# nghorbani/moshpp

Measured on NVIDIA H100. Metric: mocap frames solved/sec (Stage-II), higher is better.
Workload: dtype f32

## Files before the change

### moshpp_b200/csrc/mosh2_device.cuh

```cuda
#pragma once
#include <math.h>
#include <stdint.h>

#if defined(__CUDACC__) && !defined(MOSH2_EMU)
#define M2_HD __host__ __device__ __forceinline__
#define M2_D __device__ __forceinline__
#define M2_NOINLINE __device__ __noinline__
#define M2_SYNC() __syncthreads()
#define M2_WSYNC() __syncwarp()
#define M2_GPU 1
#else
#define M2_HD inline
#define M2_D inline
#define M2_NOINLINE static inline
#define M2_SYNC() ((void)0)
#define M2_WSYNC() ((void)0)
#define M2_GPU 0
#endif

#if defined(MOSH2_PROFILE) && M2_GPU
#define M2_T0() long long t_prev_ = clock64()
#define M2_TACC(slot) do { if (cta.tid == 0) { const long long t_now_ = clock64(); w.prof[(slot) + prof_base] += t_now_ - t_prev_; t_prev_ = t_now_; } } while (0)
#define M2_TRESET() do { t_prev_ = clock64(); } while (0)
#else
// ... 297 lines not shown
    SPtr<real> red, sc, hct;
    SPtr<int> colmap, colsrc, jlist, isc;
    SPtr<int> st_colmap, st_colsrc, st_jlist, st_meta;
    SPtr<int> c_parents, c_fk_order, c_wj, c_free1, c_free2, c_pids;
    SPtr<int> c_tin, c_tsz;
    SPtr<real> c_wv, c_v0, c_coefs, c_j0, c_hmean, c_pmeans, c_pnlw;
    SPtr<real> c_jd;
    SPtr<long long> prof;
    SPtr<uint8_t> vis;
    SPtr<uint32_t> c_chain;
    SPtr<uint8_t> c_amask;
    SPtr<unsigned long long> mbar;
    uint32_t stage_ofs, stage_bytes;
    int tc_ok;
    int tc;
};

constexpr int kMaxDepth = 16;
constexpr int kDR = 28;
constexpr int kM3 = 12;
#if M2_GPU
namespace tc {
__device__ __forceinline__ uint32_t smem_u32(const void *p) { return static_cast<uint32_t>(__cvta_generic_to_shared(p)); }
__device__ __forceinline__ uint32_t to_tf32(float v) { uint32_t r; asm("cvt.rna.tf32.f32 %0, %1;" : "=r"(r) : "f"(v)); return r; }
__device__ __forceinline__ void mma_tf32_m16n8k8(float (&d)[4], const uint32_t (&a)[4], uint32_t b0, uint32_t b1) {
    asm volatile("mma.sync.aligned.m16n8k8.row.col.f32.tf32.tf32.f32 {%0, %1, %2, %3}, {%4, %5, %6, %7}, {%8, %9}, {%0, %1, %2, %3};"
                 : "+f"(d[0]), "+f"(d[1]), "+f"(d[2]), "+f"(d[3]) : "r"(a[0]), "r"(a[1]), "r"(a[2]), "r"(a[3]), "r"(b0), "r"(b1));
}
__device__ __forceinline__ void jtj_block_tf32(const float *J, int ld, int rows, int cols, int i0, int j0,
                                               float (&hh)[2][4], float (&cr)[2][4]) {
    const int lane = threadIdx.x & 31, g = lane >> 2, t = lane & 3;
    const int ca0 = i0 + g, ca1 = i0 + 8 + g, cb0 = j0 + g, cb1 = j0 + 8 + g;
    for (int k0 = 0; k0 < rows; k0 += 8) {
        const int k1 = k0 + t, k2 = k0 + t + 4;
        const float *r1 = J + (k1 < rows ? k1 : 0) * ld, *r2 = J + (k2 < rows ? k2 : 0) * ld;
        const bool in1 = k1 < rows, in2 = k2 < rows;
        const float av[4] = {(in1 && ca0 < cols) ? r1[ca0] : 0.f, (in1 && ca1 < cols) ? r1[ca1] : 0.f,
                             (in2 && ca0 < cols) ? r2[ca0] : 0.f, (in2 && ca1 < cols) ? r2[ca1] : 0.f};
        const float bv[2][2] = {{(in1 && cb0 < cols) ? r1[cb0] : 0.f, (in2 && cb0 < cols) ? r2[cb0] : 0.f},
                                {(in1 && cb1 < cols) ? r1[cb1] : 0.f, (in2 && cb1 < cols) ? r2[cb1] : 0.f}};
        uint32_t ahi[4], alo[4], bhi[2][2], blo[2][2];
#pragma unroll
        for (int q = 0; q < 4; ++q) { ahi[q] = to_tf32(av[q]); alo[q] = to_tf32(av[q] - __uint_as_float(ahi[q])); }
#pragma unroll
        for (int nj = 0; nj < 2; ++nj)
#pragma unroll
            for (int q = 0; q < 2; ++q) { bhi[nj][q] = to_tf32(bv[nj][q]); blo[nj][q] = to_tf32(bv[nj][q] - __uint_as_float(bhi[nj][q])); }
#pragma unroll
        for (int nj = 0; nj < 2; ++nj) {
            mma_tf32_m16n8k8(hh[nj], ahi, bhi[nj][0], bhi[nj][1]);
            mma_tf32_m16n8k8(cr[nj], alo, bhi[nj][0], bhi[nj][1]);
            mma_tf32_m16n8k8(cr[nj], ahi, blo[nj][0], blo[nj][1]);
            mma_tf32_m16n8k8(cr[nj], alo, blo[nj][0], blo[nj][1]);
        }
    }
}
__device__ __forceinline__ void mbar_init(uint32_t mbar, uint32_t count) {
    asm volatile("mbarrier.init.shared::cta.b64 [%0], %1;" :: "r"(mbar), "r"(count) : "memory");
    asm volatile("fence.mbarrier_init.release.cluster;" ::: "memory");
}
__device__ __forceinline__ void mbar_wait(uint32_t mbar, uint32_t parity) {
    asm volatile("{\n\t.reg .pred p;\n\tWAIT_%=:\n\t"
                 "mbarrier.try_wait.parity.shared::cta.b64 p, [%0], %1;\n\t"
                 "@p bra DONE_%=;\n\tbra WAIT_%=;\n\tDONE_%=:\n\t}\n" :: "r"(mbar), "r"(parity) : "memory");
}
__device__ __forceinline__ void mbar_expect_tx(uint32_t mbar, uint32_t bytes) {
    asm volatile("mbarrier.arrive.expect_tx.shared::cta.b64 _, [%0], %1;" :: "r"(mbar), "r"(bytes) : "memory");
}
__device__ __forceinline__ void bulk_g2s(uint32_t dst_smem, const void *src, uint32_t bytes, uint32_t mbar) {
    asm volatile("cp.async.bulk.shared::cluster.global.mbarrier::complete_tx::bytes [%0], [%1], %2, [%3];"
                 :: "r"(dst_smem), "l"(src), "r"(bytes), "r"(mbar) : "memory");
}
__device__ __forceinline__ void fence_async_smem() { asm volatile("fence.proxy.async.shared::cta;" ::: "memory"); }
}
#endif

struct Dims {
    int nJ, M, S, PF, PR, nd, NX, NCt, n1, n2, ld, lda, ldp, npad, K, D, D4, kw, jt_size, tmk;
};

template <class real>
M2_HD Dims make_dims(const Model<real> &m) {
    Dims d;
    d.nJ = m.nJ; d.M = m.M; d.S = 3 * m.M; d.PF = 3 * m.nJ; d.PR = m.p_red; d.nd = m.nd;
    d.NX = 3 + m.p_red + m.nd; d.NCt = (m.n_hand_full + 3) & ~3;    d.n1 = m.n1; d.n2 = m.n2;
    d.npad = (m.n2 + 3) & ~3;
    d.ld = ((m.n2 + 7) & ~7) + 4;
    d.ldp = d.npad + 4;
    d.lda = d.npad | 1;
    d.K = m.prior_k; d.D = m.prior_d; d.D4 = m.prior_d4; d.kw = m.kw;
    d.tmk = m.tile_markers > 0 ? m.tile_markers : 10;
    const int a = 3 * d.tmk * d.NCt, b = kBlendGroups * 9 * m.M + 16;
    d.jt_size = a > b ? a : b;
    return d;
}

struct Arena {
    size_t off;
    template <class T> M2_HD uint32_t take(size_t n) {
        off = (off + 15) & ~size_t(15);
        const size_t o = off;
        off += n * sizeof(T);
        return uint32_t(o);
    }
};

template <class real, bool BIG>
M2_HD void carve(Work<real, BIG> &w, const Dims &d, const Model<real> &m, Arena &S, Arena &G) {
    const int hct_size = m.hct_size;
    Arena &B = BIG ? G : S;
    w.x.ofs = S.take<real>(d.NX); w.xt.ofs = S.take<real>(d.NX);
    w.pose_prev.ofs = S.take<real>(d.PR); w.velo_tgt.ofs = S.take<real>(d.PR); w.dm_tgt.ofs = S.take<real>(d.nd + 1);
    w.fullpose.ofs = S.take<real>(d.PF); w.Rl.ofs = S.take<real>(9 * d.nJ); w.dRl.ofs = S.take<real>(kDR * d.nJ);
    w.Jp.ofs = S.take<real>(3 * d.nJ); w.Rg.ofs = S.take<real>(9 * d.nJ); w.tg.ofs = S.take<real>(3 * d.nJ);
    w.vp.ofs = S.take<real>(3 * d.S); w.pj.ofs = S.take<real>(3 * d.S * d.kw); w.Rsk.ofs = S.take<real>(9 * d.S);
    w.mk.ofs = S.take<real>(3 * d.M); w.rm.ofs = S.take<real>(3 * d.M); w.obs.ofs = S.take<real>(3 * d.M);
    w.py.ofs = S.take<real>(d.K * d.D + 1); w.pq.ofs = S.take<real>(d.K + 1); w.pxg.ofs = S.take<real>(d.D + 1);
    {
        w.A.ofs = B.take<real>(size_t(d.n2) * d.lda);
        w.tc_ok = (sizeof(real) == 4 && !BIG && !m.dev_no_tc) ? 1 : 0;
        w.tc = 0;
        const size_t mark_b = B.off;
        w.Lm.ofs = B.take<real>(size_t(d.n2 + 1) * d.ld);
        const size_t end_b = B.off;
        B.off = mark_b;
        w.Jt.ofs = B.take<real>(d.jt_size);
        w.Jf.ofs = B.take<real>(3 * d.tmk * d.npad);
        if (!BIG) {
            w.Loc.ofs = S.take<real>(3 * kM3 * d.M); w.MtR.ofs = S.take<real>(kM3 * d.S);
            w.u.ofs = S.take<real>(kM3 * d.nJ); w.dtg.ofs = S.take<real>(3 * d.nJ * d.nd + 1);
        }
        if (B.off < end_b) B.off = end_b;
    }
    if (BIG) {
        w.Loc.ofs = S.take<real>(3 * kM3 * d.M); w.MtR.ofs = S.take<real>(kM3 * d.S);
        w.u.ofs = S.take<real>(kM3 * d.nJ); w.dtg.ofs = S.take<real>(3 * d.nJ * d.nd + 1);
    }
    w.Linv.ofs = S.take<real>(size_t((d.n2 + kCholNB - 1) / kCholNB) * kCholNB * kCholNB);
    w.Pn.ofs = S.take<real>(size_t(kCholNB) * d.ldp);
    w.g.ofs = S.take<real>(d.npad); w.Ag.ofs = S.take<real>(d.npad); w.dgn.ofs = S.take<real>(d.npad);
    w.d.ofs = S.take<real>(d.npad); w.tmp.ofs = S.take<real>(d.npad); w.ds.ofs = S.take<real>(d.npad);
    w.red.ofs = S.take<real>(8 * 33); w.sc.ofs = S.take<real>(16);
    w.colmap.ofs = S.take<int>(d.NX); w.colsrc.ofs = S.take<int>(d.n2); w.jlist.ofs = S.take<int>(d.nJ); w.isc.ofs = S.take<int>(8);
    w.st_colmap.ofs = S.take<int>(2 * d.NX); w.st_colsrc.ofs = S.take<int>(2 * d.n2); w.st_jlist.ofs = S.take<int>(2 * d.nJ); w.st_meta.ofs = S.take<int>(4);
    w.prof.ofs = S.take<long long>(32);
    w.mbar.ofs = S.take<unsigned long long>(1);
    w.vis.ofs = S.take<uint8_t>(d.M);
    S.off = (S.off + 15) & ~size_t(15);
    w.stage_ofs = uint32_t(S.off);
    w.c_parents.ofs = S.take<int>(d.nJ); w.c_fk_order.ofs = S.take<int>(d.nJ);
    w.c_wj.ofs = S.take<int>(d.S * d.kw); w.c_free1.ofs = S.take<int>(d.n1); w.c_free2.ofs = S.take<int>(d.n2);
    w.c_pids.ofs = S.take<int>(d.D + 1);
    w.c_wv.ofs = S.take<real>(d.S * d.kw); w.c_v0.ofs = S.take<real>(3 * d.S); w.c_coefs.ofs = S.take<real>(3 * d.M);
    w.c_j0.ofs = S.take<real>(3 * d.nJ); w.c_hmean.ofs = S.take<real>(m.n_hand_full + 1);
    w.c_pmeans.ofs = S.take<real>(d.K * d.D + 1); w.c_pnlw.ofs = S.take<real>(d.K + 1);
    w.c_jd.ofs = S.take<real>(size_t(3) * d.nJ * d.nd + 1);
    w.hct.ofs = S.take<real>(hct_size + 4);
    S.off = (S.off + 15) & ~size_t(15);
    w.stage_bytes = uint32_t(S.off) - w.stage_ofs;
    w.c_tin.ofs = S.take<int>(d.nJ); w.c_tsz.ofs = S.take<int>(d.nJ); w.c_amask.ofs = S.take<uint8_t>(size_t(d.S) * d.nJ);
    w.c_chain.ofs = S.take<uint32_t>(size_t(d.nJ) * (kMaxDepth / 4));
}

template <class real, bool BIG, class Put>
inline void stage_image(const Work<real, BIG> &w, const Dims &d, int hct_size, int n_hand_full, Put put) {
    const uint32_t b = w.stage_ofs;
    put(w.c_parents.ofs - b, 0, size_t(d.nJ)); put(w.c_fk_order.ofs - b, 1, size_t(d.nJ));
    put(w.c_wj.ofs - b, 2, size_t(d.S) * d.kw); put(w.c_free1.ofs - b, 3, size_t(d.n1)); put(w.c_free2.ofs - b, 4, size_t(d.n2));
    put(w.c_pids.ofs - b, 5, size_t(d.D));
    put(w.c_wv.ofs - b, 6, size_t(d.S) * d.kw); put(w.c_v0.ofs - b, 7, size_t(3) * d.S); put(w.c_coefs.ofs - b, 8, size_t(3) * d.M);
    put(w.c_j0.ofs - b, 9, size_t(3) * d.nJ); put(w.c_hmean.ofs - b, 10, size_t(n_hand_full));
    put(w.c_pmeans.ofs - b, 11, size_t(d.K) * d.D); put(w.c_pnlw.ofs - b, 12, size_t(d.K));
    put(w.c_jd.ofs - b, 13, size_t(3) * d.nJ * d.nd); put(w.hct.ofs - b, 14, size_t(hct_size));
}

template <class real>
struct StepCfg {
    const int *free;
    int n;
    real wp;
    real e3;
    bool velo, poseH, dm_terms, extrap;
    bool face;
};

template <class real, bool BIG = false>
struct Solver {
    const Model<real> &m;
    const Job<real> &job;
    const Work<real, BIG> &w;
    const Cta cta;
    const Dims &d;
    real wd, wp_frame, wH, wv, wdm, wex, wF, wxp;
    int nvis, njl;
    bool has_velo, has_extrap, hand_free;
    int n_iter, n_eval, n_build, n_min, frame_flags;
    int prof_base = 0;
    bool fwd_at_x = false;
    bool fwd_has_prior = false;
    bool resuming = false;
    real resume_diff = 0;
    int lin_f = -1;

    M2_D Solver(const Model<real> &m_, const Job<real> &j_, const Work<real, BIG> &w_, const Dims &d_, Cta c_)
        : m(m_), job(j_), w(w_), cta(c_), d(d_) {}

#define CTA_FOR(i, n) _Pragma("unroll 1") for (int i = cta.tid; i < (n); i += cta.nthr)

    M2_D void cta_max(real *v) {
#if M2_GPU
        real x = v[0];
#pragma unroll
        for (int o = 16; o > 0; o >>= 1) { const real y = __shfl_xor_sync(0xffffffffu, x, o); x = y > x ? y : x; }
        const int lane = cta.tid & 31, warp = cta.tid >> 5, nwarp = (cta.nthr + 31) >> 5;
        if (lane == 0) w.red[warp] = x;
        __syncthreads();
        if (cta.tid == 0) { real mx = w.red[0]; for (int q = 1; q < nwarp; ++q) mx = w.red[q] > mx ? w.red[q] : mx; w.red[32] = mx; }
        __syncthreads();
        v[0] = w.red[32];
        __syncthreads();
#else
        (void)v;
#endif
    }

    M2_D void fk(int l, int nl) {
        for (int j = l; j < d.nJ; j += nl) {
            uint32_t cw[kMaxDepth / 4];
#pragma unroll
            for (int q = 0; q < kMaxDepth / 4; ++q) cw[q] = w.c_chain[j * (kMaxDepth / 4) + q];
            int prev = int(cw[0] & 255u);
            real R[9], t[3];
#pragma unroll
            for (int i = 0; i < 9; ++i) R[i] = w.Rl[9 * prev + i];
#pragma unroll
            for (int i = 0; i < 3; ++i) t[i] = w.Jp[3 * prev + i];
#pragma unroll
            for (int k = 1; k < kMaxDepth; ++k) {
                const int c = int((cw[k >> 2] >> (8 * (k & 3))) & 255u);
                if (c != 255) {
                    const real *Rc = w.Rl + 9 * c;
                    const real dj[3] = {w.Jp[3 * c] - w.Jp[3 * prev], w.Jp[3 * c + 1] - w.Jp[3 * prev + 1], w.Jp[3 * c + 2] - w.Jp[3 * prev + 2]};
                    real rc[9], o[9];
#pragma unroll
                    for (int i = 0; i < 9; ++i) rc[i] = Rc[i];
#pragma unroll
                    for (int i = 0; i < 3; ++i) t[i] += R[3 * i] * dj[0] + R[3 * i + 1] * dj[1] + R[3 * i + 2] * dj[2];
                    mat3_mul_reg(R, rc, o);
#pragma unroll
                    for (int i = 0; i < 9; ++i) R[i] = o[i];
                    prev = c;
                }
            }
#pragma unroll
            for (int i = 0; i < 9; ++i) w.Rg[9 * j + i] = R[i];
#pragma unroll
            for (int i = 0; i < 3; ++i) w.tg[3 * j + i] = t[i];
        }
    }

    M2_D int blend_groups(int nl) const {
        const int per_group = 3 * ((d.S + 3) >> 2);
        int g = nl / per_group;
        return g < 1 ? 1 : (g > kBlendGroups ? kBlendGroups : g);
    }
    M2_D void blend_partials(int l, int nl) {
        const int G = blend_groups(nl);
        const int per = (d.nJ - 1 + G - 1) / G;
        const int Sq = (d.S + 3) >> 2;
        const size_t cs = size_t(Sq) * 4;
        for (int it = l; it < 3 * Sq * G; it += nl) {
            const int g = it / (3 * Sq), rem = it - g * 3 * Sq, c = rem / Sq, sq = rem - c * Sq;
            int j0 = 1 + g * per, j1 = j0 + per;
            if (j1 > d.nJ) j1 = d.nJ;
            real acc[4] = {0, 0, 0, 0};
            for (int j = j0; j < j1; j += 2) {
                const bool two = j + 1 < j1;
                const real *P = m.pdc + (size_t(j - 1) * 27 + c) * cs + 4 * sq, *Q = P + (two ? 27 * cs : 0);
                Vec4<real> pa[9], pb[9];
#pragma unroll
                for (int e = 0; e < 9; ++e) pa[e] = ld4(P + 3 * e * cs);
#pragma unroll
                for (int e = 0; e < 9; ++e) pb[e] = ld4(Q + 3 * e * cs);
                const real *R = w.Rl + 9 * j, *R2 = R + (two ? 9 : 0);
                const real tw = two ? real(1) : real(0);
#pragma unroll
                for (int e = 0; e < 9; ++e) {
                    const real id = (e == 0 || e == 4 || e == 8) ? real(1) : real(0);
                    const real fa = R[e] - id, fb = (R2[e] - id) * tw;
                    acc[0] += pa[e].x * fa + pb[e].x * fb;
                    acc[1] += pa[e].y * fa + pb[e].y * fb;
                    acc[2] += pa[e].z * fa + pb[e].z * fb;
                    acc[3] += pa[e].w * fa + pb[e].w * fb;
                }
            }
#pragma unroll
            for (int q = 0; q < 4; ++q) {
                const int sl = 4 * sq + q;
                if (sl < d.S) w.Jt[(g * d.S + sl) * 3 + c] = acc[q];
            }
        }
    }

    M2_D void eval(const real *xs, const StepCfg<real> &c, bool reuse = false) {
        ++n_eval;
        M2_T0();
        const real *th = xs + 3;
        const real *dl = xs + 3 + d.PR;
        if (!reuse) {
        CTA_FOR(i, d.PF) {
            real v;
            if (i < m.body_dof) {
                v = th[i];
            } else {
                const int q = i - m.body_dof;
                v = w.c_hmean[q];
                for (int b = 0; b < m.hb_n; ++b) {
                    const HandBlock hb = m.hb[b];
                    if (q >= hb.q0 && q < hb.q1) {
                        const real *ct = w.hct + hb.ct_off + (q - hb.q0) * hb.rw4;
                        for (int r = hb.r0; r < hb.r1; ++r) v += th[m.body_dof + r] * ct[r - hb.r0];
                    }
                }
            }
            w.fullpose[i] = v;
        }
        CTA_FOR(i, 3 * d.nJ) {
            real v = w.c_j0[i];
            for (int q = 0; q < d.nd; ++q) v += w.c_jd[i * d.nd + q] * dl[q];
            w.Jp[i] = v;
        }
        CTA_FOR(i, d.D) w.pxg[i] = th[w.c_pids[i]];
        M2_SYNC();
        M2_TACC(0);
#if M2_GPU
        CTA_FOR(jk, 3 * d.nJ) { const int j = jk / 3; rodrigues(w.fullpose + 3 * j, w.Rl + 9 * j, w.dRl + kDR * j, jk - 3 * j); }
#else
        CTA_FOR(j, d.nJ) rodrigues(w.fullpose + 3 * j, w.Rl + 9 * j, w.dRl + kDR * j);
#endif
        M2_SYNC();
        M2_TACC(1);
#if M2_GPU
        const int nblend = cta.nthr > 64 ? cta.nthr - 32 : cta.nthr;
        if (cta.nthr > 64) {
            if (cta.tid < 32) {
                fk(cta.tid, 32);
#if defined(MOSH2_PROFILE)
                if (cta.tid == 0) w.prof[18 + prof_base] += clock64() - t_prev_;
#endif
            } else blend_partials(cta.tid - 32, nblend);
        } else {
            fk(cta.tid, cta.nthr); __syncthreads(); blend_partials(cta.tid, nblend);
        }
#else
        const int nblend = 1;
        fk(0, 1);
        blend_partials(0, 1);
#endif
        const int nbg = blend_groups(nblend);
        M2_SYNC();
        M2_TACC(2);
        if (c.wp > real(0)) {
            const int D = d.D, D4 = d.D4;
            const real *xb = w.pxg;
#if M2_GPU
            const int nq = D4 >> 2, lchunk = (D + 3) >> 2;
            const int nitem = d.K * nq * 4, nround = (nitem + cta.nthr - 1) / cta.nthr;
#pragma unroll 1
            for (int rd = 0; rd < nround; ++rd) {
                const int it = rd * cta.nthr + cta.tid, lr = it & 3, kq = it >> 2;
                const bool on = it < nitem;
                const int k = on ? kq / nq : 0, quad = on ? kq - k * nq : 0;
                const int l0 = lr * lchunk, l1 = (l0 + lchunk < D) ? l0 + lchunk : D;
                const real *Q = m.prior_Qt + (size_t(k) * D + l0) * D4 + 4 * quad, *mu = w.c_pmeans + k * D;
                real s0 = 0, s1 = 0, s2 = 0, s3 = 0;
                for (int lb = l0; on && lb < l1; lb += 16) {
                    Vec4<real> q4[16];
#pragma unroll
                    for (int u = 0; u < 16; ++u) {
                        if (lb + u < l1) q4[u] = ld4(Q + size_t(lb + u - l0) * D4);
                        else q4[u].x = q4[u].y = q4[u].z = q4[u].w = 0;
                    }
#pragma unroll
                    for (int u = 0; u < 16; ++u) {
                        const int l = (lb + u < l1) ? lb + u : l0;
                        const real dx = xb[l] - mu[l];
                        s0 += q4[u].x * dx; s1 += q4[u].y * dx; s2 += q4[u].z * dx; s3 += q4[u].w * dx;
                    }
                }
#pragma unroll
                for (int off = 1; off <= 2; off <<= 1) {
                    s0 += __shfl_xor_sync(0xffffffffu, s0, off); s1 += __shfl_xor_sync(0xffffffffu, s1, off);
                    s2 += __shfl_xor_sync(0xffffffffu, s2, off); s3 += __shfl_xor_sync(0xffffffffu, s3, off);
                }
                if (on && lr == 0) {
                    const int i0 = 4 * quad;
                    real *o = w.py + k * D + i0;
                    if (i0 < D) o[0] = s0;
                    if (i0 + 1 < D) o[1] = s1;
                    if (i0 + 2 < D) o[2] = s2;
                    if (i0 + 3 < D) o[3] = s3;
                }
            }
#else
            for (int idx = 0; idx < d.K * D; ++idx) {
                const int k = idx / D, i = idx - k * D;
                const real *Q = m.prior_Qt + size_t(k) * D * D4 + i, *mu = w.c_pmeans + k * D;
                real s = 0;
                for (int l = 0; l < D; ++l) s += Q[size_t(l) * D4] * (xb[l] - mu[l]);
                w.py[idx] = s;
            }
#endif
        }
#if defined(MOSH2_PROFILE) && M2_GPU
        __syncthreads();
        M2_TACC(19);
#endif
        CTA_FOR(s, d.S) {
            real vpo[3];
#pragma unroll
            for (int q = 0; q < 3; ++q) vpo[q] = w.c_v0[3 * s + q];
            for (int e0 = 0; e0 < d.nd; e0 += 8) {
                real sv[24];
#pragma unroll
                for (int u = 0; u < 24; ++u) {
                    const int q = u >> 3, e = e0 + (u & 7);
                    sv[u] = e < d.nd ? m.sd[(3 * s + q) * d.nd + e] : real(0);
                }
#pragma unroll
                for (int u = 0; u < 24; ++u) {
                    const int e = e0 + (u & 7);
                    vpo[u >> 3] += sv[u] * (e < d.nd ? dl[e] : real(0));
                }
            }
            for (int q = 0; q < 3; ++q)
                for (int g = 0; g < nbg; ++g) vpo[q] += w.Jt[(g * d.S + s) * 3 + q];
            real v[3] = {0, 0, 0};
            real Rs[9] = {0, 0, 0, 0, 0, 0, 0, 0, 0};
            for (int i = 0; i < d.kw; ++i) {
                const int j = w.c_wj[s * d.kw + i];
                real *pp = w.pj + 3 * (s * d.kw + i);
                if (j < 0) { pp[0] = pp[1] = pp[2] = 0; continue; }
                const real wt = w.c_wv[s * d.kw + i];
                real dv[3] = {vpo[0] - w.Jp[3 * j], vpo[1] - w.Jp[3 * j + 1], vpo[2] - w.Jp[3 * j + 2]};
                real o[3];
                mat3_vec(w.Rg + 9 * j, dv, o);
                for (int q = 0; q < 3; ++q) {
                    pp[q] = o[q] + w.tg[3 * j + q];
                    v[q] += wt * pp[q];
                }
                for (int q = 0; q < 9; ++q) Rs[q] += wt * w.Rg[9 * j + q];
            }
            for (int q = 0; q < 3; ++q) w.vp[3 * s + q] = v[q] + xs[q];
            for (int q = 0; q < 9; ++q) w.Rsk[9 * s + q] = Rs[q];
        }
        M2_SYNC();
        M2_TACC(3);
        }
        if (reuse) {
            CTA_FOR(mi, d.M) {
                const bool vis = w.vis[mi] != 0;
                for (int q = 0; q < 3; ++q) w.rm[3 * mi + q] = vis ? (w.mk[3 * mi + q] - w.obs[3 * mi + q]) * wd : real(0);
            }
        } else
        CTA_FOR(mi, d.M) {
            const real *v0 = w.vp + 9 * mi, *v1 = v0 + 3, *v2 = v0 + 6;
            real e1[3] = {v1[0] - v0[0], v1[1] - v0[1], v1[2] - v0[2]};
            real e2[3] = {v2[0] - v0[0], v2[1] - v0[1], v2[2] - v0[2]};
            const real n1 = r_sqrt(e1[0] * e1[0] + e1[1] * e1[1] + e1[2] * e1[2]);
            real f1[3] = {e1[0] / n1, e1[1] / n1, e1[2] / n1};
            real nn[3];
            cross3(e1, e2, nn);
            const real n2 = r_sqrt(nn[0] * nn[0] + nn[1] * nn[1] + nn[2] * nn[2]);
            real f2[3] = {nn[0] / n2, nn[1] / n2, nn[2] / n2};
            real f3[3];
            cross3(f1, f2, f3);
            const real k1 = w.c_coefs[3 * mi], k2 = w.c_coefs[3 * mi + 1], k3 = w.c_coefs[3 * mi + 2];
            const bool vis = w.vis[mi] != 0;
            for (int q = 0; q < 3; ++q) {
                const real mk = v0[q] + k1 * f1[q] + k2 * f2[q] + k3 * f3[q];
                w.mk[3 * mi + q] = mk;
                w.rm[3 * mi + q] = vis ? (mk - w.obs[3 * mi + q]) * wd : real(0);
            }
        }
        M2_SYNC();
        M2_TACC(4);
        if (c.wp > real(0)) {
#if M2_GPU
            const int lane = cta.tid & 31, warp = cta.tid >> 5, nwarp = cta.nthr >> 5;
            for (int k = warp; k < d.K; k += nwarp) {
                const real *mu = w.c_pmeans + k * d.D;
                real sacc = 0;
                for (int i = lane; i < d.D; i += 32) sacc += (w.pxg[i] - mu[i]) * w.py[k * d.D + i];
                sacc = warp_sum(sacc);
                if (lane == 0) w.pq[k] = sacc + w.c_pnlw[k];
            }
#else
            for (int k = 0; k < d.K; ++k) {
                const real *mu = w.c_pmeans + k * d.D;
                real sacc = w.c_pnlw[k];
                for (int i = 0; i < d.D; ++i) sacc += (w.pxg[i] - mu[i]) * w.py[k * d.D + i];
                w.pq[k] = sacc;
            }
#endif
        }
        real part[N_ERR] = {0, 0, 0, 0, 0, 0, 0, 0};
        const int nd_dm = d.nd - m.n_expr;
        CTA_FOR(i, 3 * d.M) part[ERR_DATA] += w.rm[i] * w.rm[i];
        if (c.velo) CTA_FOR(i, d.PR) { const real e = (th[i] - w.velo_tgt[i]) * wv; part[ERR_VELO] += e * e; }
        if (c.poseH) CTA_FOR(i, m.finger_hi - m.finger_lo) { const real e = th[m.finger_lo + i] * wH; part[ERR_POSEH] += e * e; }
        if (c.wp > real(0)) CTA_FOR(i, m.n_jang) { const real e = real(2) * c.wp * r_exp(real(2) * m.jang_sign[i] * th[m.jang_id[i]]); part[ERR_POSEH] += e * e; }
        if (c.face) {
            CTA_FOR(i, m.face_hi - m.face_lo) { const real e = th[m.face_lo + i] * wF; part[ERR_POSEF] += e * e; }
            CTA_FOR(i, m.n_expr) { const real e = dl[nd_dm + i] * wxp; part[ERR_EXPR] += e * e; }
        }
        if (c.dm_terms) CTA_FOR(i, nd_dm) {
            const real e = dl[i] * wdm;
            part[ERR_DMPL] += e * e;
            if (c.extrap) { const real e2 = (dl[i] - w.dm_tgt[i]) * wex; part[ERR_EXTRAP] += e2 * e2; }
        }
        cta_reduce<real, N_ERR>(cta, part, w.red);
        if (cta.tid == 0) {
            int ks = 0;
            real sp = 0;
            if (c.wp > real(0)) {
                for (int k = 1; k < d.K; ++k) if (w.pq[k] < w.pq[ks]) ks = k;
                sp = c.wp * c.wp * w.pq[ks];
            }
            w.isc[0] = ks;
            part[ERR_POSEB] = sp;
            real tot = 0;
            for (int i = 0; i < N_ERR; ++i) { w.sc[1 + i] = part[i]; tot += part[i]; }
            w.sc[0] = tot;
        }
        M2_SYNC();
        M2_TACC(5);
    }

    M2_D void marker_local_jacobian(int mi) {
        const real *v0 = w.vp + 9 * mi, *v1 = v0 + 3, *v2 = v0 + 6;
        real e1[3] = {v1[0] - v0[0], v1[1] - v0[1], v1[2] - v0[2]};
        real e2[3] = {v2[0] - v0[0], v2[1] - v0[1], v2[2] - v0[2]};
        const real n1 = r_sqrt(e1[0] * e1[0] + e1[1] * e1[1] + e1[2] * e1[2]);
        real f1[3] = {e1[0] / n1, e1[1] / n1, e1[2] / n1};
        real nn[3];
        cross3(e1, e2, nn);
        const real n2 = r_sqrt(nn[0] * nn[0] + nn[1] * nn[1] + nn[2] * nn[2]);
        real f2[3] = {nn[0] / n2, nn[1] / n2, nn[2] / n2};
        const real k1 = w.c_coefs[3 * mi], k2 = w.c_coefs[3 * mi + 1], k3 = w.c_coefs[3 * mi + 2];
        real N1[9], Nn[9];
        for (int r = 0; r < 3; ++r)
            for (int q = 0; q < 3; ++q) {
                N1[3 * r + q] = ((r == q ? real(1) : real(0)) - f1[r] * f1[q]) / n1;
                Nn[3 * r + q] = ((r == q ? real(1) : real(0)) - f2[r] * f2[q]) / n2;
            }
        const real Se1[9] = {0, -e1[2], e1[1], e1[2], 0, -e1[0], -e1[1], e1[0], 0};
        const real Se2[9] = {0, -e2[2], e2[1], e2[2], 0, -e2[0], -e2[1], e2[0], 0};
        const real Sf1[9] = {0, -f1[2], f1[1], f1[2], 0, -f1[0], -f1[1], f1[0], 0};
        const real Sf2[9] = {0, -f2[2], f2[1], f2[2], 0, -f2[0], -f2[1], f2[0], 0};
        real df2e1[9], df2e2[9], t1[9], t2[9], df3e1[9], df3e2[9];
        mat3_mul_reg(Nn, Se2, df2e1);
        for (int q = 0; q < 9; ++q) df2e1[q] = -df2e1[q];
        mat3_mul_reg(Nn, Se1, df2e2);
        mat3_mul_reg(Sf2, N1, t1);
        mat3_mul_reg(Sf1, df2e1, t2);
        for (int q = 0; q < 9; ++q) df3e1[q] = t2[q] - t1[q];
        mat3_mul_reg(Sf1, df2e2, df3e2);
        real *L = w.Loc + 3 * kM3 * mi;
        for (int q = 0; q < 9; ++q) {
            const real de1 = k1 * N1[q] + k2 * df2e1[q] + k3 * df3e1[q];
            const real de2 = k2 * df2e2[q] + k3 * df3e2[q];
            const real id = (q == 0 || q == 4 || q == 8) ? real(1) : real(0);
            L[q] = id - de1 - de2;
            L[kM3 + q] = de1;
            L[2 * kM3 + q] = de2;
        }
    }

    M2_D void slot_mats(int sl, real (&Mt)[9], real (&Lc)[9]) {
        const real *Mp = w.MtR + kM3 * sl, *Lp = w.Loc + kM3 * sl;
        const Vec4<real> m0 = ld4(Mp), m1 = ld4(Mp + 4), m2 = ld4(Mp + 8), l0 = ld4(Lp), l1 = ld4(Lp + 4), l2 = ld4(Lp + 8);
        Mt[0] = m0.x; Mt[1] = m0.y; Mt[2] = m0.z; Mt[3] = m0.w; Mt[4] = m1.x; Mt[5] = m1.y; Mt[6] = m1.z; Mt[7] = m1.w; Mt[8] = m2.x;
        Lc[0] = l0.x; Lc[1] = l0.y; Lc[2] = l0.z; Lc[3] = l0.w; Lc[4] = l1.x; Lc[5] = l1.y; Lc[6] = l1.z; Lc[7] = l1.w; Lc[8] = l2.x;
    }

    M2_D void slot_pose_block(int sl, int a, const real (&Mt)[9], const real (&Lc)[9], const real *Pslot, real (&blk)[9]) {
        const int mask = w.c_amask[sl * d.nJ + a];
#pragma unroll
        for (int q = 0; q < 9; ++q) blk[q] = 0;
        if (a >= 1) {
            const size_t es = size_t(d.S) * 4;
            const real *P = Pslot + size_t(a - 1) * 9 * es;
            Vec4<real> pv[9];
#pragma unroll
            for (int e = 0; e < 9; ++e) pv[e] = ld4(P + e * es);
            const real *dR = w.dRl + kDR * a;
            real dr[kDR];
#pragma unroll
            for (int v = 0; v < kDR / 4; ++v) {
                const Vec4<real> q4 = ld4(dR + 4 * v);
                dr[4 * v] = q4.x; dr[4 * v + 1] = q4.y; dr[4 * v + 2] = q4.z; dr[4 * v + 3] = q4.w;
            }
            real E[9] = {0, 0, 0, 0, 0, 0, 0, 0, 0};
#pragma unroll
            for (int e = 0; e < 9; ++e) {
                const real q0 = dr[e], q1 = dr[9 + e], q2 = dr[18 + e];
                E[0] += pv[e].x * q0; E[1] += pv[e].x * q1; E[2] += pv[e].x * q2;
                E[3] += pv[e].y * q0; E[4] += pv[e].y * q1; E[5] += pv[e].y * q2;
                E[6] += pv[e].z * q0; E[7] += pv[e].z * q1; E[8] += pv[e].z * q2;
            }
#pragma unroll
            for (int r = 0; r < 3; ++r)
#pragma unroll
                for (int k = 0; k < 3; ++k)
                    blk[3 * r + k] = Mt[3 * r] * E[k] + Mt[3 * r + 1] * E[3 + k] + Mt[3 * r + 2] * E[6 + k];
        }
        if (mask) {
            real q[3] = {0, 0, 0};
            if (d.kw == 4) {
                const Vec4<real> wv = ld4(w.c_wv + 4 * sl);
                const real *pp = w.pj + 12 * sl;
                const Vec4<real> a0 = ld4(pp), a1 = ld4(pp + 4), a2 = ld4(pp + 8);
                const real g0 = w.tg[3 * a], g1 = w.tg[3 * a + 1], g2 = w.tg[3 * a + 2];
                const real w0 = (mask & 1) ? wv.x : real(0), w1 = (mask & 2) ? wv.y : real(0);
                const real w2 = (mask & 4) ? wv.z : real(0), w3 = (mask & 8) ? wv.w : real(0);
                q[0] = w0 * (a0.x - g0); q[1] = w0 * (a0.y - g1); q[2] = w0 * (a0.z - g2);
                q[0] += w1 * (a0.w - g0); q[1] += w1 * (a1.x - g1); q[2] += w1 * (a1.y - g2);
                q[0] += w2 * (a1.z - g0); q[1] += w2 * (a1.w - g1); q[2] += w2 * (a2.x - g2);
                q[0] += w3 * (a2.y - g0); q[1] += w3 * (a2.z - g1); q[2] += w3 * (a2.w - g2);
            } else
                for (int i = 0; i < d.kw; ++i)
                    if ((mask >> i) & 1) {
                        const real wt = w.c_wv[sl * d.kw + i];
                        const real *pp = w.pj + 3 * (sl * d.kw + i);
                        for (int r = 0; r < 3; ++r) q[r] += wt * (pp[r] - w.tg[3 * a + r]);
                    }
#pragma unroll
            for (int k = 0; k < 3; ++k) {
                const Vec4<real> uk = ld4(w.u + kM3 * a + 4 * k);
                const real uv[3] = {uk.x, uk.y, uk.z};
                real cr[3];
                cross3(uv, q, cr);
#pragma unroll
                for (int r = 0; r < 3; ++r) blk[3 * r + k] += Lc[3 * r] * cr[0] + Lc[3 * r + 1] * cr[1] + Lc[3 * r + 2] * cr[2];
            }
        }
    }

    M2_D void jf_store3(int ml, int col, real v0, real v1, real v2) {
        real *J = w.Jf + 3 * ml * d.npad + col;
        J[0] = v0; J[d.npad] = v1; J[2 * d.npad] = v2;
    }

    M2_D void pose_col_store(int ml, int a, int k, real sc, real b0, real b1, real b2) {
        if (3 * a < m.body_dof) {
            const int col = w.colmap[3 + 3 * a + k];
            if (col >= 0) jf_store3(ml, col, b0 * sc, b1 * sc, b2 * sc);
        } else {
            real *Jr = w.Jt + 3 * ml * d.NCt + (3 * a - m.body_dof) + k;
            Jr[0] = b0; Jr[d.NCt] = b1; Jr[2 * d.NCt] = b2;
        }
    }

    M2_D void joint_axes() {
        CTA_FOR(idx, 3 * d.nJ) {
            const int a = idx / 3, k = idx - 3 * a;
            const real *D = w.dRl + kDR * a + 9 * k, *R = w.Rl + 9 * a;
            real om[3];
            om[0] = D[6] * R[3] + D[7] * R[4] + D[8] * R[5];
            om[1] = D[0] * R[6] + D[1] * R[7] + D[2] * R[8];
            om[2] = D[3] * R[0] + D[4] * R[1] + D[5] * R[2];
            const int par = w.c_parents[a];
            real *uo = w.u + kM3 * a + 4 * k;
            if (par < 0) { for (int q = 0; q < 3; ++q) uo[q] = om[q]; }
            else mat3_vec(w.Rg + 9 * par, om, uo);
        }
    }

    M2_D void dtg_chains() {
        if (!d.nd) return;
        CTA_FOR(q, d.nJ * d.nd) {
            const int j = q / d.nd, i = q - j * d.nd;
            uint32_t cw[kMaxDepth / 4];
#pragma unroll
            for (int u = 0; u < kMaxDepth / 4; ++u) cw[u] = w.c_chain[j * (kMaxDepth / 4) + u];
            int prev = int(cw[0] & 255u);
            real acc[3];
            for (int r = 0; r < 3; ++r) acc[r] = w.c_jd[(3 * prev + r) * d.nd + i];
            for (int k = 1; k < kMaxDepth; ++k) {
                const int cj = int((cw[k >> 2] >> (8 * (k & 3))) & 255u);
                if (cj == 255) break;
                real dj[3], t[3];
                for (int r = 0; r < 3; ++r) dj[r] = w.c_jd[(3 * cj + r) * d.nd + i] - w.c_jd[(3 * prev + r) * d.nd + i];
                mat3_vec(w.Rg + 9 * prev, dj, t);
                for (int r = 0; r < 3; ++r) acc[r] = acc[r] + t[r];
                prev = cj;
            }
            real *o = w.dtg + 3 * (j * d.nd + i);
            for (int r = 0; r < 3; ++r) o[r] = acc[r];
        }
    }

    M2_D void tile_pose_columns(int t0, int tm) {
#if M2_GPU
        const int lane = cta.tid & 31, warp = cta.tid >> 5, nwarp = cta.nthr >> 5;
        const int t = lane % 3, grp = lane / 3;
        const int nmg = (tm + 9) / 10, nch = nwarp / nmg;
        const int mg = warp % nmg, ch = warp / nmg;
        const int ml = mg * 10 + grp;
        const bool valid = lane < 30 && ml < tm;
        if (ch < nch) {
            const int mi = t0 + (valid ? ml : 0), sl = 3 * mi + t;
            const real sc = (valid && w.vis[mi]) ? wd : real(0);
            real Mt[9], Lc[9];
            slot_mats(sl, Mt, Lc);
            const real *Pslot = m.pd4 + size_t(sl) * 4;
            const int src1 = lane - t + (t + 2) % 3, src2 = lane - t + (t + 1) % 3;
#pragma unroll 1
            for (int ji = ch; ji < njl; ji += nch) {
                const int a = w.jlist[ji];
                real blk[9];
                slot_pose_block(sl, a, Mt, Lc, Pslot, blk);
                real col3[3];
#pragma unroll
                for (int r = 0; r < 3; ++r) {
                    const real b0 = blk[3 * r], b1 = blk[3 * r + 1], b2 = blk[3 * r + 2];
                    const real own = sel3(t, b0, b1, b2);
                    const real to1 = sel3(t, b1, b2, b0);
                    const real to2 = sel3(t, b2, b0, b1);
                    col3[r] = own + __shfl_sync(0xffffffffu, to1, src1) + __shfl_sync(0xffffffffu, to2, src2);
                }
                if (valid) pose_col_store(ml, a, t, sc, col3[0], col3[1], col3[2]);
            }
        }
#else
        for (int gi = 0; gi < tm * njl; ++gi) {
            const int ml = gi % tm, a = w.jlist[gi / tm], mi = t0 + ml;
            real blk[9] = {0, 0, 0, 0, 0, 0, 0, 0, 0};
            for (int t = 0; t < 3; ++t) {
                const int sl = 3 * mi + t;
                real Mt[9], Lc[9], part[9];
                slot_mats(sl, Mt, Lc);
                slot_pose_block(sl, a, Mt, Lc, m.pd4 + size_t(sl) * 4, part);
                for (int q = 0; q < 9; ++q) blk[q] += part[q];
            }
            const real sc = w.vis[mi] ? wd : real(0);
            for (int k = 0; k < 3; ++k) pose_col_store(ml, a, k, sc, blk[k], blk[3 + k], blk[6 + k]);
        }
#endif
    }

    M2_D void tile_linear_columns(int t0, int tm) {
        CTA_FOR(it, tm * d.nd) {
            const int ml = it / d.nd, i = it - ml * d.nd, mi = t0 + ml;
            real val[3] = {0, 0, 0};
            real sdv[9];
#pragma unroll
            for (int u = 0; u < 9; ++u) sdv[u] = m.sd[(9 * mi + u) * d.nd + i];
            for (int t = 0; t < 3; ++t) {
                const int s = 3 * mi + t;
                real dv[3] = {0, 0, 0};
                for (int kk = 0; kk < d.kw; ++kk) {
                    const int j = w.c_wj[s * d.kw + kk];
                    if (j < 0) continue;
                    const real wt = w.c_wv[s * d.kw + kk];
                    real df[3], o[3];
                    for (int r = 0; r < 3; ++r) df[r] = sdv[3 * t + r] - w.c_jd[(3 * j + r) * d.nd + i];
                    mat3_vec(w.Rg + 9 * j, df, o);
                    for (int r = 0; r < 3; ++r) dv[r] += wt * (o[r] + w.dtg[3 * (j * d.nd + i) + r]);
                }
                const real *L = w.Loc + kM3 * s;
                for (int r = 0; r < 3; ++r) val[r] += L[3 * r] * dv[0] + L[3 * r + 1] * dv[1] + L[3 * r + 2] * dv[2];
            }
            const int col = w.colmap[3 + d.PR + i];
            const real sc = w.vis[mi] ? wd : real(0);
            if (col >= 0) jf_store3(ml, col, val[0] * sc, val[1] * sc, val[2] * sc);
        }
    }

    M2_D void tile_translation_columns(int t0, int tm, int n) {
        CTA_FOR(idx, tm * 3) {
            const int ml = idx / 3, q = idx - 3 * ml, col = w.colmap[q];
            const real v = w.vis[t0 + ml] ? wd : real(0);
            if (col >= 0) jf_store3(ml, col, q == 0 ? v : real(0), q == 1 ? v : real(0), q == 2 ? v : real(0));
        }
        const int npadc = d.npad - n;
        CTA_FOR(idx, 3 * tm * npadc) w.Jf[(idx / npadc) * d.npad + n + idx % npadc] = 0;
    }

    M2_D void tile_hand_columns(int t0, int tm) {
        if (!hand_free) return;
        int ngt = 0;
        for (int b = 0; b < m.hb_n; ++b) ngt += m.hb[b].rw4 / 4;
        CTA_FOR(it, tm * ngt) {
            const int ml = it / ngt;
            int rg = it - ml * ngt, b = 0;
            while (rg >= m.hb[b].rw4 / 4) { rg -= m.hb[b].rw4 / 4; ++b; }
            const HandBlock hb = m.hb[b];
            const int nq = hb.q1 - hb.q0;
            const real *J0 = w.Jt + 3 * ml * d.NCt + hb.q0, *J1 = J0 + d.NCt, *J2 = J1 + d.NCt;
            const real *ct = w.hct + hb.ct_off + 4 * rg;
            real acc[12] = {0, 0, 0, 0, 0, 0, 0, 0, 0, 0, 0, 0};
            constexpr int U = BIG ? 5 : 1;
            for (int q = 0; q < nq; q += U) {
                real j0[U], j1[U], j2[U];
                Vec4<real> cv[U];
#pragma unroll
                for (int u = 0; u < U; ++u) {
// ... 1218 lines not shown
```

Measured before the change: 114,000.

## Overlap pose-prior products with skinning using dedicated warps and named barriers

```diff
diff --git a/moshpp_b200/csrc/mosh2_device.cuh b/moshpp_b200/csrc/mosh2_device.cuh
--- a/moshpp_b200/csrc/mosh2_device.cuh
+++ b/moshpp_b200/csrc/mosh2_device.cuh
@@ -623,11 +623,110 @@
         }
     }
 
+    M2_D int prior_warps() const {
+#if M2_GPU
+        if (cta.nthr <= 64) return 0;
+        const int nblend = cta.nthr - 32;
+        const int idle = (nblend - 3 * ((d.S + 3) >> 2) * blend_groups(nblend)) / 32;
+        const int big = d.S > 3 * d.nJ ? d.S : 3 * d.nJ;
+        const int spare = (cta.nthr - big) / 32;
+        const int n = idle < spare ? idle : spare;
+        return n > 0 ? n : 0;
+#else
+        return 0;
+#endif
+    }
+    M2_D void bar_main(int n) const {
+#if M2_GPU
+        asm volatile("bar.sync 3, %0;" :: "r"(n) : "memory");
+#else
+        (void)n;
+#endif
+    }
+
+    M2_D void prior_products(int l, int nl) {
+        const int D = d.D, D4 = d.D4;
+        const real *xb = w.pxg;
+#if M2_GPU
+        const int nq = D4 >> 2, lchunk = (D + 3) >> 2;
+        const int nitem = d.K * nq * 4, nround = (nitem + nl - 1) / nl;
+#pragma unroll 1
+        for (int rd = 0; rd < nround; ++rd) {
+            const int it = rd * nl + l, lr = it & 3, kq = it >> 2;
+            const bool on = it < nitem;
+            const int k = on ? kq / nq : 0, quad = on ? kq - k * nq : 0;
+            const int l0 = lr * lchunk, l1 = (l0 + lchunk < D) ? l0 + lchunk : D;
+            const real *Q = m.prior_Qt + (size_t(k) * D + l0) * D4 + 4 * quad, *mu = w.c_pmeans + k * D;
+            real s0 = 0, s1 = 0, s2 = 0, s3 = 0;
+            for (int lb = l0; on && lb < l1; lb += 16) {
+                Vec4<real> q4[16];
+#pragma unroll
+                for (int u = 0; u < 16; ++u) {
+                    if (lb + u < l1) q4[u] = ld4(Q + size_t(lb + u - l0) * D4);
+                    else q4[u].x = q4[u].y = q4[u].z = q4[u].w = 0;
+                }
+#pragma unroll
+                for (int u = 0; u < 16; ++u) {
+                    const int ll = (lb + u < l1) ? lb + u : l0;
+                    const real dx = xb[ll] - mu[ll];
+                    s0 += q4[u].x * dx; s1 += q4[u].y * dx; s2 += q4[u].z * dx; s3 += q4[u].w * dx;
+                }
+            }
+#pragma unroll
+            for (int off = 1; off <= 2; off <<= 1) {
+                s0 += __shfl_xor_sync(0xffffffffu, s0, off); s1 += __shfl_xor_sync(0xffffffffu, s1, off);
+                s2 += __shfl_xor_sync(0xffffffffu, s2, off); s3 += __shfl_xor_sync(0xffffffffu, s3, off);
+            }
+            if (on && lr == 0) {
+                const int i0 = 4 * quad;
+                real *o = w.py + k * D + i0;
+                if (i0 < D) o[0] = s0;
+                if (i0 + 1 < D) o[1] = s1;
+                if (i0 + 2 < D) o[2] = s2;
+                if (i0 + 3 < D) o[3] = s3;
+            }
+        }
+#else
+        (void)l; (void)nl;
+        for (int idx = 0; idx < d.K * D; ++idx) {
+            const int k = idx / D, i = idx - k * D;
+            const real *Q = m.prior_Qt + size_t(k) * D * D4 + i, *mu = w.c_pmeans + k * D;
+            real s = 0;
+            for (int l = 0; l < D; ++l) s += Q[size_t(l) * D4] * (xb[l] - mu[l]);
+            w.py[idx] = s;
+        }
+#endif
+    }
+    M2_D void prior_energies(int wi, int nw) {
+#if M2_GPU
+        const int lane = cta.tid & 31;
+        for (int k = wi; k < d.K; k += nw) {
+            const real *mu = w.c_pmeans + k * d.D;
+            real sacc = 0;
+            for (int i = lane; i < d.D; i += 32) sacc += (w.pxg[i] - mu[i]) * w.py[k * d.D + i];
+            sacc = warp_sum(sacc);
+            if (lane == 0) w.pq[k] = sacc + w.c_pnlw[k];
+        }
+#else
+        (void)wi; (void)nw;
+        for (int k = 0; k < d.K; ++k) {
+            const real *mu = w.c_pmeans + k * d.D;
+            real sacc = w.c_pnlw[k];
+            for (int i = 0; i < d.D; ++i) sacc += (w.pxg[i] - mu[i]) * w.py[k * d.D + i];
+            w.pq[k] = sacc;
+        }
+#endif
+    }
+
     M2_D void eval(const real *xs, const StepCfg<real> &c, bool reuse = false) {
         ++n_eval;
         M2_T0();
         const real *th = xs + 3;
         const real *dl = xs + 3 + d.PR;
+        const int nmain = cta.nthr - 32 * ((!reuse && c.wp > real(0)) ? prior_warps() : 0);
+#if defined(MOSH2_PROFILE) && M2_GPU
+        long long t_pw = 0;
+#endif
         if (!reuse) {
         CTA_FOR(i, d.PF) {
             real v;
@@ -654,15 +753,24 @@
         CTA_FOR(i, d.D) w.pxg[i] = th[w.c_pids[i]];
         M2_SYNC();
         M2_TACC(0);
+#if defined(MOSH2_PROFILE) && M2_GPU
+        t_pw = clock64();
+#endif
+#if M2_GPU
+        const int nblend = cta.nthr > 64 ? cta.nthr - 32 : cta.nthr;
+#else
+        const int nblend = 1;
+#endif
+        const int nbg = blend_groups(nblend);
+        if (cta.tid < nmain) {
 #if M2_GPU
         CTA_FOR(jk, 3 * d.nJ) { const int j = jk / 3; rodrigues(w.fullpose + 3 * j, w.Rl + 9 * j, w.dRl + kDR * j, jk - 3 * j); }
 #else
         CTA_FOR(j, d.nJ) rodrigues(w.fullpose + 3 * j, w.Rl + 9 * j, w.dRl + kDR * j);
 #endif
-        M2_SYNC();
+        bar_main(nmain);
         M2_TACC(1);
 #if M2_GPU
-        const int nblend = cta.nthr > 64 ? cta.nthr - 32 : cta.nthr;
         if (cta.nthr > 64) {
             if (cta.tid < 32) {
                 fk(cta.tid, 32);
@@ -674,69 +782,20 @@
             fk(cta.tid, cta.nthr); __syncthreads(); blend_partials(cta.tid, nblend);
         }
 #else
-        const int nblend = 1;
         fk(0, 1);
         blend_partials(0, 1);
 #endif
-        const int nbg = blend_groups(nblend);
-        M2_SYNC();
+        bar_main(nmain);
         M2_TACC(2);
-        if (c.wp > real(0)) {
-            const int D = d.D, D4 = d.D4;
-            const real *xb = w.pxg;
-#if M2_GPU
-            const int nq = D4 >> 2, lchunk = (D + 3) >> 2;
-            const int nitem = d.K * nq * 4, nround = (nitem + cta.nthr - 1) / cta.nthr;
-#pragma unroll 1
-            for (int rd = 0; rd < nround; ++rd) {
-                const int it = rd * cta.nthr + cta.tid, lr = it & 3, kq = it >> 2;
-                const bool on = it < nitem;
-                const int k = on ? kq / nq : 0, quad = on ? kq - k * nq : 0;
-                const int l0 = lr * lchunk, l1 = (l0 + lchunk < D) ? l0 + lchunk : D;
-                const real *Q = m.prior_Qt + (size_t(k) * D + l0) * D4 + 4 * quad, *mu = w.c_pmeans + k * D;
-                real s0 = 0, s1 = 0, s2 = 0, s3 = 0;
-                for (int lb = l0; on && lb < l1; lb += 16) {
-                    Vec4<real> q4[16];
-#pragma unroll
-                    for (int u = 0; u < 16; ++u) {
-                        if (lb + u < l1) q4[u] = ld4(Q + size_t(lb + u - l0) * D4);
-                        else q4[u].x = q4[u].y = q4[u].z = q4[u].w = 0;
-                    }
-#pragma unroll
-                    for (int u = 0; u < 16; ++u) {
-                        const int l = (lb + u < l1) ? lb + u : l0;
-                        const real dx = xb[l] - mu[l];
-                        s0 += q4[u].x * dx; s1 += q4[u].y * dx; s2 += q4[u].z * dx; s3 += q4[u].w * dx;
-                    }
-                }
-#pragma unroll
-                for (int off = 1; off <= 2; off <<= 1) {
-                    s0 += __shfl_xor_sync(0xffffffffu, s0, off); s1 += __shfl_xor_sync(0xffffffffu, s1, off);
-                    s2 += __shfl_xor_sync(0xffffffffu, s2, off); s3 += __shfl_xor_sync(0xffffffffu, s3, off);
-                }
-                if (on && lr == 0) {
-                    const int i0 = 4 * quad;
-                    real *o = w.py + k * D + i0;
-                    if (i0 < D) o[0] = s0;
-                    if (i0 + 1 < D) o[1] = s1;
-                    if (i0 + 2 < D) o[2] = s2;
-                    if (i0 + 3 < D) o[3] = s3;
-                }
-            }
-#else
-            for (int idx = 0; idx < d.K * D; ++idx) {
-                const int k = idx / D, i = idx - k * D;
-                const real *Q = m.prior_Qt + size_t(k) * D * D4 + i, *mu = w.c_pmeans + k * D;
-                real s = 0;
-                for (int l = 0; l < D; ++l) s += Q[size_t(l) * D4] * (xb[l] - mu[l]);
-                w.py[idx] = s;
-            }
-#endif
+        }
+        {
+            const int p0 = nmain < cta.nthr ? nmain : 0;
+            if (c.wp > real(0) && cta.tid >= p0) prior_products(cta.tid - p0, cta.nthr - p0);
         }
 #if defined(MOSH2_PROFILE) && M2_GPU
-        __syncthreads();
-        M2_TACC(19);
-#endif
+        if (nmain == cta.nthr) { __syncthreads(); M2_TACC(19); }
+#endif
+        if (cta.tid < nmain) {
         CTA_FOR(s, d.S) {
             real vpo[3];
 #pragma unroll
@@ -775,15 +834,8 @@
             for (int q = 0; q < 3; ++q) w.vp[3 * s + q] = v[q] + xs[q];
             for (int q = 0; q < 9; ++q) w.Rsk[9 * s + q] = Rs[q];
         }
-        M2_SYNC();
+        bar_main(nmain);
         M2_TACC(3);
-        }
-        if (reuse) {
-            CTA_FOR(mi, d.M) {
-                const bool vis = w.vis[mi] != 0;
-                for (int q = 0; q < 3; ++q) w.rm[3 * mi + q] = vis ? (w.mk[3 * mi + q] - w.obs[3 * mi + q]) * wd : real(0);
-            }
-        } else
         CTA_FOR(mi, d.M) {
             const real *v0 = w.vp + 9 * mi, *v1 = v0 + 3, *v2 = v0 + 6;
             real e1[3] = {v1[0] - v0[0], v1[1] - v0[1], v1[2] - v0[2]};
@@ -804,27 +856,26 @@
                 w.rm[3 * mi + q] = vis ? (mk - w.obs[3 * mi + q]) * wd : real(0);
             }
         }
+        } else {
+#if M2_GPU
+        asm volatile("bar.sync 4, %0;" :: "r"(cta.nthr - nmain) : "memory");
+#endif
+        }
+        }
+        else
+        CTA_FOR(mi, d.M) {
+            const bool vis = w.vis[mi] != 0;
+            for (int q = 0; q < 3; ++q) w.rm[3 * mi + q] = vis ? (w.mk[3 * mi + q] - w.obs[3 * mi + q]) * wd : real(0);
+        }
+        {
+            const int p0 = nmain < cta.nthr ? nmain : 0;
+            if (c.wp > real(0) && cta.tid >= p0) prior_energies((cta.tid - p0) >> 5, (cta.nthr - p0) >> 5);
+        }
+#if defined(MOSH2_PROFILE) && M2_GPU
+        if (nmain < cta.nthr && cta.tid == nmain) w.prof[19 + prof_base] += clock64() - t_pw;
+#endif
         M2_SYNC();
         M2_TACC(4);
-        if (c.wp > real(0)) {
-#if M2_GPU
-            const int lane = cta.tid & 31, warp = cta.tid >> 5, nwarp = cta.nthr >> 5;
-            for (int k = warp; k < d.K; k += nwarp) {
-                const real *mu = w.c_pmeans + k * d.D;
-                real sacc = 0;
-                for (int i = lane; i < d.D; i += 32) sacc += (w.pxg[i] - mu[i]) * w.py[k * d.D + i];
-                sacc = warp_sum(sacc);
-                if (lane == 0) w.pq[k] = sacc + w.c_pnlw[k];
-            }
-#else
-            for (int k = 0; k < d.K; ++k) {
-                const real *mu = w.c_pmeans + k * d.D;
-                real sacc = w.c_pnlw[k];
-                for (int i = 0; i < d.D; ++i) sacc += (w.pxg[i] - mu[i]) * w.py[k * d.D + i];
-                w.pq[k] = sacc;
-            }
-#endif
-        }
         real part[N_ERR] = {0, 0, 0, 0, 0, 0, 0, 0};
         const int nd_dm = d.nd - m.n_expr;
         CTA_FOR(i, 3 * d.M) part[ERR_DATA] += w.rm[i] * w.rm[i];
```

After: 116,000 (median of 6 runs). +1.7%, better.
